# Sachin-A/TraceWeaver

Hardware: AMD Instinct MI355X
Metric: spans/sec reconstructed + assignment accuracy vs ground truth (higher is better)
Workload: dtype int64 timestamps, f64 scores; 1 GPU; media_microservices shape (6 services, E in {1,1,1,1,2,4}), 100000 requests/service x 16 replicas per GPU, concurrency 1.6, two-pass reconstruction, device mixture refit; spans_per_gpu=25600000, spans_total=25600000, parallelism=units sharded, 1 rank(s), backend none

## Files before the change

traceweaver_amd/csrc/tw_device.h:

```cpp
#pragma once
#include <hip/hip_runtime.h>
#include <stdint.h>

#include "traceweaver_amd.h"

namespace tw {

constexpr int kMaxEp = TW_MAX_EP;
constexpr int kTopK = TW_TOPK;
constexpr int kMaxComp = TW_MAX_COMP;
constexpr int kMaxWin = TW_MAX_WINDOW;
constexpr int kCandWords = TW_CAND_WORDS;
constexpr int kEnumStretches = 8;
constexpr int kTile = 128;
constexpr int kCoop = 256;
constexpr int32_t kNoOwner = 0x7f7f7f7f;

struct UnitDev {
    int64_t in_off;
    int64_t ie_off;
    int64_t ep_off[kMaxEp + 1];
    int32_t n_in;
    int32_t E;
    int32_t nblk;
// ... 91 lines not shown
    int32_t *heavy_in_unit, *heavy_in_idx;
    int32_t* heavy_big_count;
    int32_t *heavy_big_unit, *heavy_big_idx;
    int32_t heavy_big_off[kMaxEp + 2];
    int32_t* heavy_big_part;
    int32_t* heavy_big_slot;
    int32_t part_off[kMaxEp + 2];
    int32_t split_twins;
    int32_t* part_used;
    int32_t defer_min_e;
    int32_t defer_cap;
    unsigned long long* defer_list;
    int32_t* defer_used;
    int32_t* defer_count;
    int32_t *part_lo, *part_hi;
    int32_t* part_lvl;
    int32_t* any_wide;
    int32_t* redo_count;
    int32_t* defer_refused;
    int32_t lean_min_e;
    int32_t tile_max_deep;
    int32_t lean_grid;
    int32_t tile_rank;
    double* pair_pool;
    int32_t* pair_busy;
    int32_t* fb_count;
    int32_t* fb_total;
    int32_t *fb_unit, *fb_idx, *fb_part, *fb_slot;
    int32_t* split_count;
    int32_t *split_unit, *split_idx, *split_slot, *split_parts;
    int32_t* part_n;
    int64_t* part_leaves;
    double* part_score;
    int32_t* part_idx;
    unsigned long long* part_bits;
    int32_t* part_logn;
    double* part_log_sc;
    unsigned long long* part_log_ix;
    int32_t* err;
    unsigned long long* prof;
};

__device__ __forceinline__ int32_t hi_word(double x) { return (int32_t)(__double_as_longlong(x) >> 32); }
__device__ __forceinline__ uint32_t lo_word(double x) { return (uint32_t)__double_as_longlong(x); }
__device__ __forceinline__ double with_hi(double x, int32_t hi) {
    return __longlong_as_double((long long)(((uint64_t)(uint32_t)hi << 32) | (uint64_t)lo_word(x)));
// ... 199 lines not shown
```

traceweaver_amd/csrc/tw_engine.hip:

```cpp
#include <algorithm>
#include <chrono>
#include <cmath>
#include <cstdio>
#include <cstdlib>
#include <cstring>
#include <functional>
#include <string>
#include <type_traits>
#include <vector>

#include <hip/hip_runtime.h>
#include <rocprim/rocprim.hpp>

#include "traceweaver_amd.h"
#include "tw_kernels.h"
#include "tw_fit.h"
#include "tw_eval.h"
#include "tw_skip.h"
#include "tw_load.h"
#include "tw_baselines.h"
#include "tw_stitch.h"
#include "tw_attr.h"
#include "tw_conf.h"
#include "tw_dist.h"
// ... 60 lines not shown
    hipEvent_t stretch_ev[kMaxEp + 1][kEnumStretches] = {}, stretch_done[kMaxEp + 1] = {};
    int enum_stretches = 1, stretch_min_tiles = 2048;
    int heavy_grid = 4096, select_grid = 0;
    int debug_lists = 0;
    int32_t first_lists[3][kMaxEp + 1] = {};
    hipEvent_t gate_ev = nullptr;
    int tile_gate = 0;
    int stage_min_tiles = 1024;
    int32_t *rank_in = nullptr, *rank_out = nullptr;
    bool class_params = false;
    int prio_min_e = 0, prio_high = 0;
    bool prio_any = false;
    int pipeline = 1;
    std::string err;
    int state = ST_EMPTY;
    int tile = kTile;
    int tile_threads = 2;
    int tile_single = 1;
    int tile_rank = 1;
    int block_params = 1;
    int tile_single_threads = 1;
    int tile_pair = 1;
    int tile_pair_threads = 2;
    int coop = kCoop;
    std::vector<UnitDev> units;
    std::vector<TileDev> tiles;
    std::vector<int64_t> gs_off_h;
    std::vector<void*> allocs;
    void* arena = nullptr;
    size_t arena_cap = 0;
    bool arena_open = false;
    std::vector<std::pair<std::function<void(void*)>, size_t>> arena_req;
    Dev P{};
    int64_t n_ie = 0, n_gp = 0, n_slots = 0, n_gaps = 0;
    PairVI* agg_pair = nullptr;
    int32_t *agg_i32 = nullptr, *agg_i32b = nullptr;
    uint32_t *seg_in = nullptr, *seg_out = nullptr;
    int n_seg_out = 0;
    void* sort_tmp = nullptr;
    size_t sort_tmp_bytes = 0;
    double* mix_p_dev = nullptr;
    int32_t* mix_n_dev = nullptr;
    double* mix_c_dev = nullptr;
    double* gaps_sorted = nullptr;
    double* fit_models = nullptr;
    double* fit_uval = nullptr;
// ... 305 lines not shown
    const int pool = E > 4 ? 2048 : (E > 1 ? kPairPoolPerEp * E : 1);
    const size_t pool_bytes = sizeof(double) * (size_t)pool;
    const size_t lean_bytes = sizeof(double) * (size_t)(2 * kMaxEp * kNarrow + e->lean_pool), lean_bytes_w = sizeof(double) * (size_t)(2 * kMaxEp * 64 * kCandWords + e->lean_pool);
    const bool lean = E >= P.lean_min_e && !e->skip_mode;
    const int cap = P.heavy_in_off[E + 1] - P.heavy_in_off[E];
    auto grid_for = [&](int known, int most) { return std::max(std::min(((known >= 0 ? known : cap) + kWorkChunk - 1) / kWorkChunk, most), 1); };
    auto narrow = [&](int part, int g) {
        if (lean) hipLaunchKernelGGL((k_enumerate_lean<kNarrow>), dim3(g), hb, lean_bytes, st, P, pass, mode, part, e->lean_pool, E, E);
        else hipLaunchKernelGGL((k_enumerate_heavy<E, kNarrow>), dim3(g), hb, pool_bytes, st, P, pass, mode, part, pool);
    };
    auto wide = [&](int part, int g) {
        if (lean) hipLaunchKernelGGL((k_enumerate_lean<64 * kCandWords>), dim3(g), hb, lean_bytes_w, st, P, pass, mode, part, e->lean_pool, E, E);
        else hipLaunchKernelGGL((k_enumerate_heavy<E, 64 * kCandWords>), dim3(g), hb, pool_bytes, st, P, pass, mode, part, pool);
    };
    bool stretched = false;
    if (mode == 0 && pass == 1 && e->class_params) {
        const TileSet S = class_tiles(e, E);
        (void)sort_ends(e, S, st);
        launch_block_params(e, E, st);
    }
    if (mode == 0) {
        const bool single = E == 1 && e->tile_single != 0;
        const bool pair = E == 2 && e->tile_pair != 0;
        const dim3 tile_block(e->tile >= 64 ? e->tile * (single ? e->tile_single_threads : (pair ? e->tile_pair_threads : e->tile_threads)) : e->tile);
        int sub = 1;
        while (sub < e->tile_sub_max && nt * sub < 512 && (e->tile / (sub * 2)) * (sub * 2) == e->tile && e->tile / (sub * 2) >= 8) sub *= 2;
        const int ns = (!lean && !e->skip_mode && !(E >= 3 && E >= P.defer_min_e) && e->cls_stream2[E] != nullptr)
                           ? std::max(std::min(e->enum_stretches, nt / e->stretch_min_tiles), 1) : 1;
        stretched = ns > 1;
        for (int j = 0; j < ns; j++) {
            const int t0 = (int)((int64_t)nt * j / ns), t1 = (int)((int64_t)nt * (j + 1) / ns);
            const int32_t* ids = e->tile_ids + e->tile_cls_off[E] + t0;
            const bool sub_tile = e->tile == kTile && e->tile / sub == kSubTileSpans;
            if constexpr (E == 1) {
                if (single && sub_tile) hipLaunchKernelGGL((k_enumerate_tile<1, kSubTileSpans, true>), dim3((t1 - t0) * sub), tile_block, 0, st, P, pass, ids, t1 - t0, sub);
                else if (single) hipLaunchKernelGGL((k_enumerate_tile<1, kTile, true>), dim3((t1 - t0) * sub), tile_block, 0, st, P, pass, ids, t1 - t0, sub);
            }
            if constexpr (E == 2) {
                if (pair && sub_tile) hipLaunchKernelGGL((k_enumerate_tile<2, kSubTileSpans, false, true>), dim3((t1 - t0) * sub), tile_block, 0, st, P, pass, ids, t1 - t0, sub);
                else if (pair) hipLaunchKernelGGL((k_enumerate_tile<2, kTile, false, true>), dim3((t1 - t0) * sub), tile_block, 0, st, P, pass, ids, t1 - t0, sub);
            }
            if (single || pair) {}
            else if (sub_tile)
                hipLaunchKernelGGL((k_enumerate_tile<E, kSubTileSpans>), dim3((t1 - t0) * sub), tile_block, 0, st, P, pass, ids, t1 - t0, sub);
            else
                hipLaunchKernelGGL((k_enumerate_tile<E>), dim3((t1 - t0) * sub), tile_block, 0, st, P, pass, ids, t1 - t0, sub);
            if (ns > 1) {
                hipLaunchKernelGGL(k_enum_snapshot, dim3(1), dim3(1), 0, st, P, E, j + 1);
                if (j + 1 < ns) {
                    hipStream_t s2 = e->cls_stream2[E];
                    (void)hipEventRecord(e->stretch_ev[E][j], st);
                    (void)hipStreamWaitEvent(s2, e->stretch_ev[E][j], 0);
                    hipLaunchKernelGGL((k_enumerate_heavy<E, kNarrow>), dim3(grid_for(-1, e->heavy_grid)), hb, pool_bytes, s2, P, pass, mode, (j + 1) << 8, pool);
                } else {
                    hipLaunchKernelGGL((k_enumerate_heavy<E, kNarrow>), dim3(grid_for(-1, e->heavy_grid)), hb, pool_bytes, st, P, pass, mode, (j + 1) << 8, pool);
                    (void)hipEventRecord(e->stretch_done[E], e->cls_stream2[E]);
                    (void)hipStreamWaitEvent(st, e->stretch_done[E], 0);
                }
            }
        }
        if (e->tile_gate > 0 && nt >= e->tile_gate) { (void)hipEventRecord(e->tile_ev[E], st); e->gate_ev = e->tile_ev[E]; }
    }
    if (n_narrow != 0 && !stretched) narrow(0, grid_for(n_narrow, e->heavy_grid));
    if (n_wide != 0) wide(0, grid_for(n_wide, 1024));
    if (mode == 0 && E >= 3 && E >= P.defer_min_e) { narrow(3, grid_for(-1, 4096)); if (n_wide != 0) wide(3, grid_for(-1, 1024)); }
// ... 443 lines not shown
    HIPCHK(hipMemcpyAsync(const_cast<UnitDev*>(P.units), e->units.data(), sizeof(UnitDev) * e->units.size(), hipMemcpyHostToDevice, e->stream));
    HIPCHK(hipStreamSynchronize(e->stream));
    e->state = ST_LOADED; e->pass1_done = false;
    drop_batch_order(e);
    for (int E = 0; E <= kMaxEp; E++) { e->wide_pass1[E] = -1; e->hard_pass1[E] = -1; e->split_pass1[E] = -1; }
    return TW_OK;
}

extern "C" {

int tw_create(int device_id, tw_engine** out) {
    if (out == nullptr) return TW_ERR_ARG;
    *out = nullptr;
    tw_engine* e = new tw_engine();
    e->device = device_id;
    e->tile = std::min(std::max(env_int("TW_TILE", kTile), 1), kTile);
    e->tile_threads = std::min(std::max(env_int("TW_TILE_THREADS", 2), 1), 4);
    e->tile_single = env_int("TW_TILE_SINGLE", 1);
    e->block_params = env_int("TW_BLOCK_PARAMS", 1);
    e->tile_rank = env_int("TW_TILE_RANK", 1) != 0 ? 1 : 0;
    e->tile_single_threads = std::min(std::max(env_int("TW_TILE_SINGLE_THREADS", 1), 1), 4);
    e->tile_pair = env_int("TW_TILE_PAIR", 1);
    e->tile_pair_threads = std::min(std::max(env_int("TW_TILE_PAIR_THREADS", 2), 1), 2);
    e->coop = std::min(std::max(env_int("TW_COOP_THREADS", kCoop), 1), kCoop);
    if (env_int("TW_SET_HW_QUEUES", 0) != 0) setenv("GPU_MAX_HW_QUEUES", "12", 0);
    hipError_t s = hipSetDevice(device_id);
    if (s == hipSuccess) s = hipStreamCreate(&e->stream);
    for (int i = 0; i < EV_COUNT && s == hipSuccess; i++) s = hipEventCreate(&e->ev[i]);
    for (int i = 0; i < SE_COUNT && s == hipSuccess; i++) s = hipEventCreate(&e->stage_ev[i]);
    const int prio_min_e = env_int("TW_PRIO_MIN_E", 0);
    int prio_least = 0, prio_greatest = 0;
    if (s == hipSuccess) s = hipDeviceGetStreamPriorityRange(&prio_least, &prio_greatest);
    e->prio_min_e = prio_min_e; e->prio_high = prio_greatest; e->prio_any = prio_greatest != prio_least;
    for (int i = 0; i <= kMaxEp + 1 && s == hipSuccess; i++) s = hipEventCreateWithFlags(&e->cls_ev[i], hipEventDisableTiming);
    if (s == hipSuccess) s = hipEventCreateWithFlags(&e->prep_ev, hipEventDisableTiming);
    for (int i = 0; i <= kMaxEp && s == hipSuccess; i++) {
        s = hipEventCreateWithFlags(&e->post_fork[i], hipEventDisableTiming);
        if (s == hipSuccess) s = hipEventCreateWithFlags(&e->tile_ev[i], hipEventDisableTiming);
        if (s == hipSuccess) s = hipEventCreateWithFlags(&e->post_done[i], hipEventDisableTiming);
        if (s == hipSuccess) s = hipEventCreateWithFlags(&e->stretch_done[i], hipEventDisableTiming);
        for (int j = 0; j < kEnumStretches && s == hipSuccess; j++) s = hipEventCreateWithFlags(&e->stretch_ev[i][j], hipEventDisableTiming);
        for (int j = 0; j < 3 && s == hipSuccess; j++) s = hipEventCreateWithFlags(&e->post_join[i][j], hipEventDisableTiming);
    }
    e->pipeline = env_int("TW_CLASS_PIPELINE", 1);
    e->sig_hash_bits = std::min(std::max(env_int("TW_SIG_HASH_BITS", 64), 1), 64);
    e->tile_gate = env_int("TW_TILE_GATE", 0);
// ... 209 lines not shown
    std::vector<uint32_t> seg_gap_dst_h(seg_gap_h.size());
    e->n_gap_scored = 0;
    for (size_t r = 0; r < seg_gap_h.size(); r++) { seg_gap_dst_h[r] = (uint32_t)e->n_gap_scored; e->n_gap_scored += seg_gap_end_h[r] - seg_gap_h[r]; }
    seg_in[(size_t)b->n_units] = (uint32_t)n_in_total;
    seg_out.push_back((uint32_t)n_out_total);
    e->n_seg_out = (int)seg_out.size() - 1;
    e->n_ie = ie; e->n_gp = gp; e->n_slots = slots; e->n_gaps = gaps;

    Dev& P = e->P;
    P = Dev{};
    P.n_units = b->n_units;
    P.n_tiles = (int32_t)e->tiles.size();
    P.tile_spans = e->tile;
    P.n_in_total = n_in_total;
    P.n_out_total = n_out_total;
    P.batch_size = b->batch_size;
    P.batch_mis = b->batch_size_mis;
    P.split_twins = env_int("TW_SPLIT_TWINS", 2);
    P.defer_min_e = env_int("TW_DEFER_MIN_E", 5);
    P.lean_min_e = env_int("TW_LEAN_MIN_E", 5);
    P.lean_grid = std::max(env_int("TW_LEAN_GRID", TW_LEAN_GRID), 1);
    P.tile_max_deep = std::min(std::max(env_int("TW_TILE_MAX_DEEP", kTileMax), 0), kTileMax);
    P.tile_rank = e->tile_rank;
    int rc;
    e->arena_req.clear();
    e->arena_open = true;
    UnitDev* d_units; TileDev* d_tiles; int64_t *d_is, *d_ie, *d_os, *d_oe, *d_gs;
    DEV_ALLOC(d_units, P.n_units); DEV_ALLOC(d_tiles, P.n_tiles);
    DEV_ALLOC(d_is, n_in_total); DEV_ALLOC(d_ie, n_in_total); DEV_ALLOC(d_os, n_out_total); DEV_ALLOC(d_oe, n_out_total);
    DEV_ALLOC(d_gs, P.n_units);
    DEV_ALLOC(P.in_end_sorted, n_in_total); DEV_ALLOC(P.out_end_sorted, n_out_total);
    DEV_ALLOC(P.gparam, gp * 4);
    DEV_ALLOC(e->mix_n_dev, slots); DEV_ALLOC(e->mix_p_dev, slots * kMaxComp * 3); DEV_ALLOC(e->mix_c_dev, slots * kMaxComp * 4);
    DEV_ALLOC(P.pm_val, n_in_total); DEV_ALLOC(P.pm_idx, n_in_total); DEV_ALLOC(P.pc, n_in_total + 1); DEV_ALLOC(P.seg, n_in_total);
    DEV_ALLOC(P.win_end, n_in_total); DEV_ALLOC(P.wid, n_in_total); DEV_ALLOC(P.w_last, n_in_total);
    DEV_ALLOC(P.unit_nwin, P.n_units); DEV_ALLOC(P.w_dirty, n_in_total); DEV_ALLOC(P.w_conf, n_in_total);
    DEV_ALLOC(P.tk_n, n_in_total); DEV_ALLOC(P.leaves, n_in_total); DEV_ALLOC(P.leaves0, n_in_total); DEV_ALLOC(P.chosen, n_in_total); DEV_ALLOC(P.rep, n_in_total);
    DEV_ALLOC(P.tkr_n, n_in_total);
    DEV_ALLOC(P.tk_idx, ie * kTopK); DEV_ALLOC(P.tkr_idx, ie * kTopK);
    DEV_ALLOC(P.tk_score, n_in_total * kTopK); DEV_ALLOC(P.tkr_score, n_in_total * kTopK);
    DEV_ALLOC(P.c_lo, ie); DEV_ALLOC(P.c_hi, ie); DEV_ALLOC(P.c_bits, ie * kCandWords); DEV_ALLOC(P.parent, ie);
    DEV_ALLOC(P.gone, ie * kCandWords); DEV_ALLOC(P.gone_valid, n_in_total); DEV_ALLOC(P.leaves_r, n_in_total);
    DEV_ALLOC(P.frontier, (int64_t)kFrontierSlots * 2 * kFrontierCap); 
    P.frontier_big_slots = (int32_t)std::min<int64_t>(std::max<int64_t>(n_in_total / 16384, kFrontierBigSlots), std::max(kFrontierBigSlots, 512));
    DEV_ALLOC(P.frontier_big, (int64_t)P.frontier_big_slots * 2 * kFrontierBigCap);
    DEV_ALLOC(P.pair_pool, (int64_t)kPairSlots * kPairSpill);
// ... 1812 lines not shown
```

traceweaver_amd/csrc/tw_tile.h:

```cpp
#pragma once

namespace tw {

#ifndef TW_TILE_MAX
#define TW_TILE_MAX 256
#endif
constexpr int kTileMax = TW_TILE_MAX;
#ifndef TW_TILE_REPLAY_MAX
#define TW_TILE_REPLAY_MAX 256
#endif
constexpr int kTileReplayMax = TW_TILE_REPLAY_MAX;
#ifndef TW_TILE_RANK_DIRECT
#define TW_TILE_RANK_DIRECT 32
#endif
constexpr int kRankDirect = TW_TILE_RANK_DIRECT;
constexpr int kRankMinLong = (kRankDirect & ~3) + 4;
constexpr int kRankBuckets = 5;
static_assert(kRankDirect >= 24, "the maxima and counters of a segment's long spans lie in one byte per tuple slot");
__device__ __forceinline__ uint32_t score_key32(double v) {
    const unsigned long long u = (unsigned long long)__double_as_longlong(v + 0.0);
    return (uint32_t)(((u >> 63) ? ~u : (u | (1ull << 63))) >> 32);
}
__device__ __forceinline__ int pos_base(unsigned long long pk, int e) {
    int acc = 0;
    for (int f = 0; f < e; f++) acc += (int)((pk >> (8 * f)) & 255ull);
    return acc;
}
#ifndef TW_TILE_ITEMS
#define TW_TILE_ITEMS 768
#define TW_TILE_GRID 1024
#endif
constexpr int kSubTileSpans = kTile / 8;
#ifndef TW_TILE_PAIR_ITEMS
#define TW_TILE_PAIR_ITEMS 512
#define TW_TILE_PAIR_GRID 1024
#endif
template <int E, int SPANS = kTile, bool PAIR = false>
struct TileCfg {
#ifdef TW_TILE_SMALL
    static constexpr int kSlice = 24, kItems = PAIR ? 2 * 32 : kMaxEp * 32, kGrid = kTileMax > 64 ? kTileMax : 64;
#else
    static constexpr int kSlice = SPANS < kTile ? 64 : (E <= 4 ? 192 : 160);
    static constexpr int kItems = SPANS < kTile ? kMaxEp * 32 : (PAIR ? TW_TILE_PAIR_ITEMS : TW_TILE_ITEMS);
    static constexpr int kGrid = SPANS < kTile ? (kTileMax > 512 ? kTileMax : 512) : (PAIR ? TW_TILE_PAIR_GRID : TW_TILE_GRID);
#endif
    static_assert(kItems >= (PAIR ? 2 : kMaxEp) * 32 && kGrid >= ((kTileMax + 3) & ~3) && kGrid % 4 == 0, "a single span must fit a segment");
};

__device__ __forceinline__ uint32_t div_small(uint32_t rest, uint32_t c) {
#ifdef TW_HOST_EMULATION
    const float rc = 1.0f / (float)c;
#else
    const float rc = __builtin_amdgcn_rcpf((float)c);
#endif
    return (uint32_t)(((float)rest + 0.5f) * rc);
}

__device__ __forceinline__ int fresh(int v) {
#ifndef TW_HOST_EMULATION
    asm volatile("" : "+v"(v));
#endif
    return v;
}

template <int GRID, int MINLONG>
struct SurvivorRanks {
    static constexpr int kLong = (GRID - MINLONG) / MINLONG + 1;
// ... 94 lines not shown
#ifndef TW_PROFILE_TILE_E
#define TW_PROFILE_TILE_E 4
#endif
#define TW_TILE_T0() long long _tp = wall_clock64(); const long long _tb = _tp; long long _ta[7] = {0, 0, 0, 0, 0, 0, 0}
#define TW_TILE_TICK(k) do { const long long _n = wall_clock64(); _ta[k] += _n - _tp; _tp = _n; } while (0)
#define TW_TILE_COUNT(k, v) do { if (E == TW_PROFILE_TILE_E && threadIdx.x == 0) atomicAdd((unsigned long long*)&P.prof[k], (unsigned long long)(v)); } while (0)
#define TW_TILE_FLUSH() do { if (E == TW_PROFILE_TILE_E && threadIdx.x == 0) { for (int _k = 0; _k < 7; _k++) atomicAdd((unsigned long long*)&P.prof[_k], (unsigned long long)_ta[_k]); \
    atomicAdd((unsigned long long*)&P.prof[7], (unsigned long long)(wall_clock64() - _tb)); atomicAdd((unsigned long long*)&P.prof[8], 1ull); } } while (0)
#else
#define TW_TILE_T0() do {} while (0)
#define TW_TILE_TICK(k) do {} while (0)
#define TW_TILE_COUNT(k, v) do {} while (0)
#define TW_TILE_FLUSH() do {} while (0)
#endif

#ifdef TW_HOST_EMULATION
#define TW_TILE_ATTR
#else
#ifndef TW_TILE_PAIR_WAVES
#define TW_TILE_PAIR_WAVES 4
#endif
#define TW_TILE_ATTR __attribute__((amdgpu_waves_per_eu(SINGLE ? 8 : (PAIR ? TW_TILE_PAIR_WAVES : (E <= 4 ? 4 : 2)))))
#endif
template <int E, int SPANS = kTile, bool SINGLE = false, bool PAIR = false>
__global__ void __launch_bounds__(4 * kTile) TW_TILE_ATTR k_enumerate_tile(Dev P, int pass, const int32_t* tile_ids, int n_tiles_e, int sub_tiles) {
    static_assert(!SINGLE || E == 1, "the lean path is the one of a single endpoint");
    static_assert(!PAIR || (E == 2 && !SINGLE), "the pair path is the one of two endpoints");
    if (*P.err != 0) return;
    typedef TileCfg<E, SPANS, PAIR> C;
    constexpr int SL = C::kSlice;
    const int vb = xcd_tile(blockIdx.x, n_tiles_e * sub_tiles);
    const int tile = tile_ids[vb / sub_tiles];
    const TileDev T = P.tiles[tile];
    const UnitDev& U = P.units[T.unit];
    const int t = threadIdx.x, nt = blockDim.x;
    const int sub_spans = P.tile_spans / sub_tiles, first = T.first + (vb % sub_tiles) * sub_spans;
    const int ns = min(sub_spans, min(P.tile_spans, U.n_in - T.first) - (vb % sub_tiles) * sub_spans);
    if (ns <= 0) return;
    __shared__ int32_t s_is[SPANS], s_ie[SPANS];
    __shared__ int32_t sl_st[E][SL], sl_en[E][SL];
    __shared__ int32_t s_A[E], s_B[E];
    __shared__ uint16_t s_lo[E][SPANS];
    __shared__ uint32_t s_cm[E][SPANS];
    __shared__ uint32_t s_bits[E][SPANS];
    __shared__ int32_t s_item0[SPANS + 1], s_grid0[SPANS + 1], s_leaves[SPANS];
    __shared__ uint8_t s_amb[SPANS];
    __shared__ unsigned long long s_cn[SPANS];
    __shared__ int32_t s_wtot[4 * kTile / 64][2];
    __shared__ double t_root[C::kItems], t_close[C::kItems];
    __shared__ uint16_t it_idx[C::kItems];
    __shared__ double g_sc[C::kGrid + (PAIR ? 4 : 0)];
    __shared__ uint8_t g_span[C::kGrid];
    __shared__ uint32_t g_aux[C::kGrid / 4];
    __shared__ int32_t s_segend, s_anyamb;
    const bool live = t < ns;
    const int i = first + (live ? t : 0);
    const int64_t base = P.in_start[U.in_off + first];
    const int64_t in_start = P.in_start[U.in_off + i], in_end = P.in_end[U.in_off + i];
    const int64_t* os[E];
    const int64_t* oe[E];
#pragma unroll
    for (int e = 0; e < E; e++) { os[e] = P.out_start + U.ep_off[e]; oe[e] = P.out_end + U.ep_off[e]; }
    for (int x = t; x < E; x += nt) { s_A[x] = 0x7fffffff; s_B[x] = 0; }
    uint32_t dag_pm[E], dag_np[E], dag_pl[E];
    uint32_t ordered = 0;
#pragma unroll
    for (int e = 0; e < E; e++) {
        dag_pm[e] = U.pred_mask[e];
        dag_np[e] = U.npred[e];
        uint32_t pk = 0;
#pragma unroll
        for (int j = 0; j < E; j++) pk |= (j < (int)dag_np[e] ? ((uint32_t)U.pred_list[e][j] | ((uint32_t)U.pred_prim[e][j] << 3)) : 0u) << (4 * j);
        dag_pl[e] = pk;
        ordered |= dag_pm[e];
    }
// ... 108 lines not shown
                } else {
                    int64_t prev = INT64_MIN;
                    for (int cx = lo[e]; cx <= hi[e]; cx++) {
                        const int64_t st = os[e][cx];
                        if (st >= in_start && oe[e][cx] <= in_end) { v++; twins |= st == prev; prev = st; }
                    }
                }
                if (hprod <= (1ll << 40)) hprod *= v;
                if (e == 0) first_cands = v;
            }
            if (twins && P.split_twins == 0) first_cands = 0;
            twins_any = twins;
            if (E >= P.lean_min_e) first_cands = 0;
            if (E >= 3 && E >= P.defer_min_e) {
                uint32_t any_order = 0;
#pragma unroll
                for (int e = 0; e < E; e++) any_order |= U.pred_mask[e];
                if (any_order != 0) first_cands = 0;
            }
        }
        heavy_append<E>(P, live && !mine && !wide, narrow, hprod > kBigProduct, T.unit, i, hprod, U.skip ? 0 : first_cands, twins_any);
    }
    const bool some = mine && !empty && prod > 0;
    int nitem = 0;
    unsigned long long cnpack = 0;
    if (live) {
#pragma unroll
        for (int e = 0; e < E; e++) {
            const int rel = lo[e] - s_A[e], c = some ? __popcll((unsigned long long)cm[e]) : 0;
            s_lo[e][t] = (uint16_t)(some ? rel : 0);
            s_cm[e][t] = some ? cm[e] : 0u;
            if constexpr (!SINGLE) s_bits[e][t] = 0u;
            nitem += c;
            cnpack |= (unsigned long long)c << (8 * e);
        }
        s_is[t] = (int32_t)iso; s_ie[t] = (int32_t)ieo;
        s_amb[t] = 0;
        if constexpr (!SINGLE) { s_cn[t] = cnpack; s_leaves[t] = (some && !ordered) ? (int)prod : 0; }
    }
    {
        int a = live ? nitem : 0, b = (!SINGLE && live && some) ? (PAIR ? (int)prod : (((int)prod + 3) & ~3)) : 0;
        const int lane = t & 63, wv = t >> 6;
        for (int off = 1; off < 64; off <<= 1) {
            const int a2 = __shfl_up(a, off);
            if (lane >= off) a += a2;
            if constexpr (!SINGLE) { const int b2 = __shfl_up(b, off); if (lane >= off) b += b2; }
        }
        if (lane == 63 || t == nt - 1) { s_wtot[wv][0] = a; if constexpr (!SINGLE) s_wtot[wv][1] = b; }
        group_sync();
        for (int w = 0; w < wv; w++) { a += s_wtot[w][0]; if constexpr (!SINGLE) b += s_wtot[w][1]; }
        if (live) { s_item0[t + 1] = a; if constexpr (!SINGLE) s_grid0[t + 1] = b; }
        if (t == 0) { s_item0[0] = 0; if constexpr (!SINGLE) s_grid0[0] = 0; }
        group_sync();
    }
    TW_TILE_TICK(2);
    Scorer S;
    S.pass = pass;
    S.mix_n = P.mix_n + U.slot_off;
    S.mix_c = P.mix_c + (int64_t)U.slot_off * kMaxComp * 4;
    auto span_of = [&](const int32_t* pre, int first, int last, int x) -> int {
        int a = first, b = last - 1;
        while (a < b) { const int mid = (a + b + 1) >> 1; if (pre[mid] <= x) a = mid; else b = mid - 1; }
        return a;
    };
    auto decode = [&](int s, int gi, int it_first, int32_t (&kx)[E], int32_t (&ix)[E]) {
        uint32_t rest = (uint32_t)gi;
        const unsigned long long pk = s_cn[s];
        int below[E], acc = s_item0[s] - it_first;
#pragma unroll
        for (int e = 0; e < E; e++) { below[e] = acc; acc += (int)((pk >> (8 * e)) & 255ull); }
#pragma unroll
        for (int e = E - 1; e >= 0; e--) {
            const uint32_t c = (uint32_t)((pk >> (8 * e)) & 255ull);
            const uint32_t q = c == 1 ? rest : div_small(rest, c);
            kx[e] = below[e] + (int32_t)(rest - q * c);
// ... 283 lines not shown
                for (int k = 0; k < kTopK; k++) { hs[k] = RH.s[k]; hx[k] = (uint16_t)RH.x[k]; }
                py_sort_desc(hs, hx, RH.n, [&](double sa, unsigned long long xa, double sb, unsigned long long xb) { return RH.lt(sa, xa, sb, xb, start_of); });
                const int si = first + tl;
                for (int k = 0; k < RH.n; k++) {
                    P.tk_score[tks_index(U, k, si)] = hs[k];
                    P.tk_idx[tk_index(U, k, 0, si)] = s_A[0] + (int)it_idx[ks + (int)(hx[k] & 255u)];
                    P.tk_idx[tk_index(U, k, 1, si)] = s_A[1] + (int)(it_idx[ks + c0 + (int)(hx[k] >> 8)] & 0x7fff);
                }
                s_amb[tl] = 0;
            }
            if (mine_here && !s_amb[tl]) {
                const int i = first + tl;
                const int64_t g = U.in_off + i;
                const int leaves = s_leaves[tl];
                P.tk_n[g] = leaves < kTopK ? leaves : kTopK;
                P.leaves[g] = leaves;
                if (pass == 1) P.leaves0[g] = leaves;
                P.rep[g] = 0;
                if (pass == 1) {
#pragma unroll
                    for (int e = 0; e < 2; e++) {
                        P.c_bits[ie_index(U, e, i) * kCandWords] = (uint64_t)(ordered ? s_bits[e][tl] : s_cm[e][tl]);
                        for (int w = 1; w < kCandWords; w++) P.c_bits[ie_index(U, e, i) * kCandWords + w] = 0;
                    }
                }
            }
            group_sync();
            TW_TILE_TICK(6);
            seg = send;
        }
        TW_TILE_FLUSH();
        const int te = fresh(t);
        heavy_append<E>(P, te < ns && s_mine[te] != 0 && s_amb[te] != 0, true, false, T.unit, first + (te < ns ? te : 0), 0, 0, false, te & 63);
        return;
    } else
    for (int seg = 0; seg < ns;) {
        typedef SurvivorRanks<C::kGrid, kRankMinLong> SR;
        constexpr bool kRankFits = SR::kAuxWords <= C::kGrid / 4 && C::kGrid * 4 <= C::kItems * 8 && C::kGrid <= 65536;
        static_assert(kRankBuckets == kTopK && C::kGrid <= C::kItems * 8, "a subset of slots per entry of the list; a rank per slot in t_root");
        uint8_t* const g_rank = reinterpret_cast<uint8_t*>(t_root);
        const bool compact = kRankFits && P.tile_rank != 0;
        if (compact) SR{g_aux, g_rank, nullptr, nullptr, g_sc, g_span, s_grid0, 0}.clear(fresh(t), nt);
        if (t == 0) { s_segend = ns; s_anyamb = 0; }
        group_sync();
        if (live && t >= seg && (s_item0[t + 1] - s_item0[seg] > C::kItems || s_grid0[t + 1] - s_grid0[seg] > C::kGrid)) atomicMin(&s_segend, t);
        group_sync();
// ... 210 lines not shown
```

Measured before the change: 1.382 billion spans/s.

## Add specialized quad tile enumeration path for three- and four-endpoint spans

Adds a QUAD specialization of the tile enumeration kernel for units with three or four endpoints, enabled by default. It precomputes per-item root and closing gap scores as a compacted job list, and prunes closing candidates that cannot be the last-ending endpoint. Scores per tuple then reuse these precomputed terms. The kernel also gets its own item and grid sizes and unpadded grid counts. This removes redundant per-tuple scoring for the E=4 service, at the cost of more shared memory, an extra prefix scan, and a large new code path that could diverge from the generic one in results.

```diff
diff --git a/traceweaver_amd/csrc/tw_device.h b/traceweaver_amd/csrc/tw_device.h
--- a/traceweaver_amd/csrc/tw_device.h
+++ b/traceweaver_amd/csrc/tw_device.h
@@ -137,6 +137,7 @@
     int32_t tile_max_deep;
     int32_t lean_grid;
     int32_t tile_rank;
+    int32_t tile_quad_close;
     double* pair_pool;
     int32_t* pair_busy;
     int32_t* fb_count;
diff --git a/traceweaver_amd/csrc/tw_engine.hip b/traceweaver_amd/csrc/tw_engine.hip
--- a/traceweaver_amd/csrc/tw_engine.hip
+++ b/traceweaver_amd/csrc/tw_engine.hip
@@ -106,6 +106,8 @@
     int tile_single_threads = 1;
     int tile_pair = 1;
     int tile_pair_threads = 2;
+    int tile_quad = 1;
+    int tile_quad_close = 1;
     int coop = kCoop;
     std::vector<UnitDev> units;
     std::vector<TileDev> tiles;
@@ -457,6 +459,7 @@
     if (mode == 0) {
         const bool single = E == 1 && e->tile_single != 0;
         const bool pair = E == 2 && e->tile_pair != 0;
+        const bool quad = (E == 3 || E == 4) && e->tile_quad != 0;
         const dim3 tile_block(e->tile >= 64 ? e->tile * (single ? e->tile_single_threads : (pair ? e->tile_pair_threads : e->tile_threads)) : e->tile);
         int sub = 1;
         while (sub < e->tile_sub_max && nt * sub < 512 && (e->tile / (sub * 2)) * (sub * 2) == e->tile && e->tile / (sub * 2) >= 8) sub *= 2;
@@ -475,7 +478,11 @@
                 if (pair && sub_tile) hipLaunchKernelGGL((k_enumerate_tile<2, kSubTileSpans, false, true>), dim3((t1 - t0) * sub), tile_block, 0, st, P, pass, ids, t1 - t0, sub);
                 else if (pair) hipLaunchKernelGGL((k_enumerate_tile<2, kTile, false, true>), dim3((t1 - t0) * sub), tile_block, 0, st, P, pass, ids, t1 - t0, sub);
             }
-            if (single || pair) {}
+            if constexpr (E == 3 || E == 4) {
+                if (quad && sub_tile) hipLaunchKernelGGL((k_enumerate_tile<E, kSubTileSpans, false, false, true>), dim3((t1 - t0) * sub), tile_block, 0, st, P, pass, ids, t1 - t0, sub);
+                else if (quad) hipLaunchKernelGGL((k_enumerate_tile<E, kTile, false, false, true>), dim3((t1 - t0) * sub), tile_block, 0, st, P, pass, ids, t1 - t0, sub);
+            }
+            if (single || pair || quad) {}
             else if (sub_tile)
                 hipLaunchKernelGGL((k_enumerate_tile<E, kSubTileSpans>), dim3((t1 - t0) * sub), tile_block, 0, st, P, pass, ids, t1 - t0, sub);
             else
@@ -965,6 +972,8 @@
     e->tile_single_threads = std::min(std::max(env_int("TW_TILE_SINGLE_THREADS", 1), 1), 4);
     e->tile_pair = env_int("TW_TILE_PAIR", 1);
     e->tile_pair_threads = std::min(std::max(env_int("TW_TILE_PAIR_THREADS", 2), 1), 2);
+    e->tile_quad = env_int("TW_TILE_QUAD", 1);
+    e->tile_quad_close = env_int("TW_TILE_QUAD_CLOSE", 1) != 0 ? 1 : 0;
     e->coop = std::min(std::max(env_int("TW_COOP_THREADS", kCoop), 1), kCoop);
     if (env_int("TW_SET_HW_QUEUES", 0) != 0) setenv("GPU_MAX_HW_QUEUES", "12", 0);
     hipError_t s = hipSetDevice(device_id);
@@ -1220,6 +1229,7 @@
     P.lean_grid = std::max(env_int("TW_LEAN_GRID", TW_LEAN_GRID), 1);
     P.tile_max_deep = std::min(std::max(env_int("TW_TILE_MAX_DEEP", kTileMax), 0), kTileMax);
     P.tile_rank = e->tile_rank;
+    P.tile_quad_close = e->tile_quad_close;
     int rc;
     e->arena_req.clear();
     e->arena_open = true;
diff --git a/traceweaver_amd/csrc/tw_tile.h b/traceweaver_amd/csrc/tw_tile.h
--- a/traceweaver_amd/csrc/tw_tile.h
+++ b/traceweaver_amd/csrc/tw_tile.h
@@ -35,14 +35,18 @@
 #define TW_TILE_PAIR_ITEMS 512
 #define TW_TILE_PAIR_GRID 1024
 #endif
-template <int E, int SPANS = kTile, bool PAIR = false>
+#ifndef TW_TILE_QUAD_ITEMS
+#define TW_TILE_QUAD_ITEMS 512
+#define TW_TILE_QUAD_GRID 1024
+#endif
+template <int E, int SPANS = kTile, bool PAIR = false, bool QUAD = false>
 struct TileCfg {
 #ifdef TW_TILE_SMALL
     static constexpr int kSlice = 24, kItems = PAIR ? 2 * 32 : kMaxEp * 32, kGrid = kTileMax > 64 ? kTileMax : 64;
 #else
     static constexpr int kSlice = SPANS < kTile ? 64 : (E <= 4 ? 192 : 160);
-    static constexpr int kItems = SPANS < kTile ? kMaxEp * 32 : (PAIR ? TW_TILE_PAIR_ITEMS : TW_TILE_ITEMS);
-    static constexpr int kGrid = SPANS < kTile ? (kTileMax > 512 ? kTileMax : 512) : (PAIR ? TW_TILE_PAIR_GRID : TW_TILE_GRID);
+    static constexpr int kItems = SPANS < kTile ? kMaxEp * 32 : (PAIR ? TW_TILE_PAIR_ITEMS : (QUAD ? TW_TILE_QUAD_ITEMS : TW_TILE_ITEMS));
+    static constexpr int kGrid = SPANS < kTile ? (kTileMax > 512 ? kTileMax : 512) : (PAIR ? TW_TILE_PAIR_GRID : (QUAD ? TW_TILE_QUAD_GRID : TW_TILE_GRID));
 #endif
     static_assert(kItems >= (PAIR ? 2 : kMaxEp) * 32 && kGrid >= ((kTileMax + 3) & ~3) && kGrid % 4 == 0, "a single span must fit a segment");
 };
@@ -183,12 +187,13 @@
 #endif
 #define TW_TILE_ATTR __attribute__((amdgpu_waves_per_eu(SINGLE ? 8 : (PAIR ? TW_TILE_PAIR_WAVES : (E <= 4 ? 4 : 2)))))
 #endif
-template <int E, int SPANS = kTile, bool SINGLE = false, bool PAIR = false>
+template <int E, int SPANS = kTile, bool SINGLE = false, bool PAIR = false, bool QUAD = false>
 __global__ void __launch_bounds__(4 * kTile) TW_TILE_ATTR k_enumerate_tile(Dev P, int pass, const int32_t* tile_ids, int n_tiles_e, int sub_tiles) {
     static_assert(!SINGLE || E == 1, "the lean path is the one of a single endpoint");
     static_assert(!PAIR || (E == 2 && !SINGLE), "the pair path is the one of two endpoints");
     if (*P.err != 0) return;
-    typedef TileCfg<E, SPANS, PAIR> C;
+    static_assert(!QUAD || ((E == 3 || E == 4) && !SINGLE && !PAIR), "the quad path is the one of three and four endpoints");
+    typedef TileCfg<E, SPANS, PAIR, QUAD> C;
     constexpr int SL = C::kSlice;
     const int vb = xcd_tile(blockIdx.x, n_tiles_e * sub_tiles);
     const int tile = tile_ids[vb / sub_tiles];
@@ -205,13 +210,14 @@
     __shared__ uint32_t s_cm[E][SPANS];
     __shared__ uint32_t s_bits[E][SPANS];
     __shared__ int32_t s_item0[SPANS + 1], s_grid0[SPANS + 1], s_leaves[SPANS];
+    __shared__ int32_t s_job0[QUAD ? SPANS + 1 : 1];
     __shared__ uint8_t s_amb[SPANS];
     __shared__ unsigned long long s_cn[SPANS];
-    __shared__ int32_t s_wtot[4 * kTile / 64][2];
+    __shared__ int32_t s_wtot[4 * kTile / 64][QUAD ? 3 : 2];
     __shared__ double t_root[C::kItems], t_close[C::kItems];
     __shared__ uint16_t it_idx[C::kItems];
-    __shared__ double g_sc[C::kGrid + (PAIR ? 4 : 0)];
-    __shared__ uint8_t g_span[C::kGrid];
+    __shared__ double g_sc[C::kGrid + (PAIR || QUAD ? 4 : 0)];
+    __shared__ uint8_t g_span[C::kGrid] __attribute__((aligned(4)));
     __shared__ uint32_t g_aux[C::kGrid / 4];
     __shared__ int32_t s_segend, s_anyamb;
     const bool live = t < ns;
@@ -366,8 +372,36 @@
         heavy_append<E>(P, live && !mine && !wide, narrow, hprod > kBigProduct, T.unit, i, hprod, U.skip ? 0 : first_cands, twins_any);
     }
     const bool some = mine && !empty && prod > 0;
-    int nitem = 0;
+    int nitem = 0, njob = 0;
     unsigned long long cnpack = 0;
+    uint32_t clm[QUAD ? E : 1];
+    if constexpr (QUAD) {
+#pragma unroll
+        for (int e = 0; e < E; e++) clm[e] = some ? cm[e] : 0u;
+        if (some && !ordered && P.tile_quad_close != 0) {
+            int32_t mn[E];
+#pragma unroll
+            for (int e = 0; e < E; e++) {
+                const int rel = lo[e] - s_A[e];
+                mn[e] = 0x7fffffff;
+                for (uint32_t m = cm[e]; m != 0; m &= m - 1) { const int32_t en = sl_en[e][rel + __ffs((int)m) - 1]; mn[e] = en < mn[e] ? en : mn[e]; }
+            }
+#pragma unroll
+            for (int e = 0; e < E; e++) {
+                const int rel = lo[e] - s_A[e];
+                int32_t above = -0x7fffffff - 1, reach = -0x7fffffff - 1;
+#pragma unroll
+                for (int f = 0; f < E; f++) { if (f < e && mn[f] > above) above = mn[f]; if (f > e && mn[f] > reach) reach = mn[f]; }
+                uint32_t keep = 0;
+                for (uint32_t m = cm[e]; m != 0; m &= m - 1) {
+                    const int r = __ffs((int)m) - 1;
+                    const int32_t en = sl_en[e][rel + r];
+                    if (en > above && en >= reach) keep |= 1u << r;
+                }
+                clm[e] = keep;
+            }
+        }
+    }
     if (live) {
 #pragma unroll
         for (int e = 0; e < E; e++) {
@@ -375,6 +409,10 @@
             s_lo[e][t] = (uint16_t)(some ? rel : 0);
             s_cm[e][t] = some ? cm[e] : 0u;
             if constexpr (!SINGLE) s_bits[e][t] = 0u;
+            if constexpr (QUAD) {
+                if (!ordered) s_bits[e][t] = clm[e];
+                njob += (dag_np[e] == 0 ? c : 0) + __popcll((unsigned long long)clm[e]);
+            }
             nitem += c;
             cnpack |= (unsigned long long)c << (8 * e);
         }
@@ -383,18 +421,21 @@
         if constexpr (!SINGLE) { s_cn[t] = cnpack; s_leaves[t] = (some && !ordered) ? (int)prod : 0; }
     }
     {
-        int a = live ? nitem : 0, b = (!SINGLE && live && some) ? (PAIR ? (int)prod : (((int)prod + 3) & ~3)) : 0;
+        int a = live ? nitem : 0, b = (!SINGLE && live && some) ? (PAIR || QUAD ? (int)prod : (((int)prod + 3) & ~3)) : 0;
+        int c = live ? njob : 0;
         const int lane = t & 63, wv = t >> 6;
         for (int off = 1; off < 64; off <<= 1) {
             const int a2 = __shfl_up(a, off);
             if (lane >= off) a += a2;
             if constexpr (!SINGLE) { const int b2 = __shfl_up(b, off); if (lane >= off) b += b2; }
-        }
-        if (lane == 63 || t == nt - 1) { s_wtot[wv][0] = a; if constexpr (!SINGLE) s_wtot[wv][1] = b; }
+            if constexpr (QUAD) { const int c2 = __shfl_up(c, off); if (lane >= off) c += c2; }
+        }
+        if (lane == 63 || t == nt - 1) { s_wtot[wv][0] = a; if constexpr (!SINGLE) s_wtot[wv][1] = b; if constexpr (QUAD) s_wtot[wv][2] = c; }
         group_sync();
-        for (int w = 0; w < wv; w++) { a += s_wtot[w][0]; if constexpr (!SINGLE) b += s_wtot[w][1]; }
-        if (live) { s_item0[t + 1] = a; if constexpr (!SINGLE) s_grid0[t + 1] = b; }
-        if (t == 0) { s_item0[0] = 0; if constexpr (!SINGLE) s_grid0[0] = 0; }
+        for (int w = 0; w < wv; w++) { a += s_wtot[w][0]; if constexpr (!SINGLE) b += s_wtot[w][1]; if constexpr (QUAD) c += s_wtot[w][2]; }
+        if (live) { s_item0[t + 1] = a; if constexpr (!SINGLE) s_grid0[t + 1] = b; if constexpr (QUAD) s_job0[t + 1] = c; }
+        if (t == 0) { s_item0[0] = 0; if constexpr (!SINGLE) s_grid0[0] = 0; if constexpr (QUAD) s_job0[0] = 0; }
+        (void)c;
         group_sync();
     }
     TW_TILE_TICK(2);
@@ -724,6 +765,268 @@
                     for (int e = 0; e < 2; e++) {
                         P.c_bits[ie_index(U, e, i) * kCandWords] = (uint64_t)(ordered ? s_bits[e][tl] : s_cm[e][tl]);
                         for (int w = 1; w < kCandWords; w++) P.c_bits[ie_index(U, e, i) * kCandWords + w] = 0;
+                    }
+                }
+            }
+            group_sync();
+            TW_TILE_TICK(6);
+            seg = send;
+        }
+        TW_TILE_FLUSH();
+        const int te = fresh(t);
+        heavy_append<E>(P, te < ns && s_mine[te] != 0 && s_amb[te] != 0, true, false, T.unit, first + (te < ns ? te : 0), 0, 0, false, te & 63);
+        return;
+    } else if constexpr (QUAD) {
+        static_assert(SL <= 256 && E <= 4, "the slice positions of a tuple's candidates lie in a byte each of 32 bits");
+        static_assert(C::kItems <= (1 << 14), "an item's number in 15 bits of a job, its endpoint above 14 bits of it_idx");
+        __shared__ uint8_t it_span[C::kItems];
+        __shared__ uint32_t g_ix[C::kGrid];
+        __shared__ uint8_t s_row[C::kGrid / 64 + 1];
+        __shared__ uint8_t s_mine[SPANS];
+        if (live) s_mine[t] = mine ? 1 : 0;
+        uint16_t* const jobs = reinterpret_cast<uint16_t*>(g_sc);
+        constexpr int kJobs = 2 * C::kItems < 4 * C::kGrid ? 2 * C::kItems : 4 * C::kGrid;
+        static_assert(kJobs >= 2 * E * 32, "the jobs of a single span must fit a segment");
+        typedef SurvivorRanks<C::kGrid, kRankDirect + 1> SR;
+        constexpr bool kRankFits = SR::kAuxWords <= C::kGrid / 4 && C::kGrid * 4 <= C::kItems * 8 && C::kGrid <= 65536;
+        static_assert(C::kGrid <= C::kItems * 8, "a rank per slot in t_root");
+        uint8_t* const g_rank = reinterpret_cast<uint8_t*>(t_root);
+        const bool compact = kRankFits && P.tile_rank != 0;
+        const bool scan = (nt & 63) == 0;
+        for (int seg = 0; seg < ns;) {
+            if (compact) SR{g_aux, g_rank, nullptr, nullptr, g_sc, g_span, s_grid0, 0}.clear(fresh(t), nt);
+            for (int x = fresh(t); x < C::kGrid / 4; x += nt) reinterpret_cast<uint32_t*>(g_span)[x] = 0u;
+            if (t == 0) { s_segend = ns; s_anyamb = 0; }
+            group_sync();
+            if (live && t >= seg && (s_item0[t + 1] - s_item0[seg] > C::kItems || s_grid0[t + 1] - s_grid0[seg] > C::kGrid || (kJobs < 2 * C::kItems && s_job0[t + 1] - s_job0[seg] > kJobs))) atomicMin(&s_segend, t);
+            group_sync();
+            const int send = s_segend;
+            const int it0 = s_item0[seg], nIt = s_item0[send] - it0, g0 = s_grid0[seg], nG = s_grid0[send] - g0, j0 = s_job0[seg], nJ = s_job0[send] - j0;
+            const SR sr{g_aux, g_rank, reinterpret_cast<uint16_t*>(t_close), reinterpret_cast<uint16_t*>(t_close) + C::kGrid, g_sc, g_span, s_grid0, g0};
+            const int tq = fresh(t);
+            const bool here = tq < ns && tq >= seg && tq < send;
+            TW_TILE_TICK(2);
+            TW_TILE_COUNT(9, 1); TW_TILE_COUNT(10, nIt); TW_TILE_COUNT(11, nG); TW_TILE_COUNT(12, nJ);
+            if (here) {
+                int k = s_item0[tq] - it0, j = s_job0[tq] - j0;
+#pragma unroll
+                for (int e = 0; e < E; e++) {
+                    const int rel = s_lo[e][tq];
+                    const bool is_root = dag_np[e] == 0;
+                    const uint32_t cl = ordered ? s_cm[e][tq] : s_bits[e][tq];
+                    for (uint32_t m = s_cm[e][tq]; m != 0; m &= m - 1, k++) {
+                        const int r = __ffs((int)m) - 1;
+                        it_span[k] = (uint8_t)tq;
+                        it_idx[k] = (uint16_t)((rel + r) | (e << 14));
+                        if (is_root) jobs[j++] = (uint16_t)k;
+                        if ((cl >> r) & 1u) jobs[j++] = (uint16_t)(k | 0x8000);
+                        else t_close[k] = dnan();
+                    }
+                }
+                const int gs = s_grid0[tq] - g0, ge = s_grid0[tq + 1] - g0;
+                if (ge > gs) {
+                    g_span[gs] = (uint8_t)tq;
+                    for (int r = (gs + 63) >> 6; (r << 6) < ge; r++) s_row[r] = (uint8_t)tq;
+                }
+            }
+            group_sync();
+            for (int j = t; j < nJ; j += nt) {
+                const int jb = jobs[j], k = jb & 0x7fff;
+                const bool closing = (jb >> 15) != 0;
+                const int s = it_span[k], e = it_idx[k] >> 14, idx = it_idx[k] & 255;
+                const long long gap = closing ? (long long)s_ie[s] - sl_en[e][idx] : (long long)sl_st[e][idx] - s_is[s];
+                S.gp = P.gparam + (U.gp_off + (int64_t)((first + s) / P.batch_size) * U.nslot) * 4;
+                const double v = score_term_gap(S, closing ? slot_close(E, e) : slot_root(E, e), gap);
+                (closing ? t_close : t_root)[k] = v;
+            }
+            group_sync();
+            TW_TILE_TICK(3);
+            for (int gb = 0; gb < nG; gb += nt) {
+                const int g = gb + t;
+                int s = 0;
+                if (scan) {
+                    const int lane = t & 63;
+                    if (g < nG) { s = g_span[g]; if (lane == 0) { const int c = s_row[g >> 6]; s = c > s ? c : s; } }
+                    for (int off = 1; off < 64; off <<= 1) { const int s2 = __shfl_up(s, off); if (lane >= off && s2 > s) s = s2; }
+                } else if (g < nG) s = span_of(s_grid0, seg, send, g0 + g);
+                if (g >= nG) continue;
+                const int gi = g - (s_grid0[s] - g0);
+                const uint32_t pk = (uint32_t)s_cn[s];
+                int32_t kx[E], ix[E], st[E], en[E];
+                {
+                    uint32_t rest = (uint32_t)gi;
+                    int below[E], acc = s_item0[s] - it0;
+#pragma unroll
+                    for (int e = 0; e < E; e++) { below[e] = acc; acc += (int)((pk >> (8 * e)) & 255u); }
+#pragma unroll
+                    for (int e = E - 1; e >= 0; e--) {
+                        const uint32_t c = (pk >> (8 * e)) & 255u;
+                        const uint32_t q = e == 0 ? 0u : (c == 1 ? rest : div_small(rest, c));
+                        kx[e] = below[e] + (int32_t)(rest - q * c);
+                        rest = q;
+                        ix[e] = it_idx[kx[e]] & 255;
+                    }
+                }
+                bool ok = true;
+#pragma unroll
+                for (int e = 0; e < E; e++) {
+                    st[e] = sl_st[e][ix[e]]; en[e] = sl_en[e][ix[e]];
+#pragma unroll
+                    for (int p = 0; p < e; p++)
+                        if (((dag_pm[e] >> p) & 1) && en[p] > st[e]) ok = false;
+                }
+                double sj = 0.0;
+                if (ok) {
+                    int last = 0;
+                    int32_t last_end = en[0];
+#pragma unroll
+                    for (int e = 1; e < E; e++) if (en[e] > last_end) { last_end = en[e]; last = e; }
+                    if (ordered) S.gp = P.gparam + (U.gp_off + (int64_t)((first + s) / P.batch_size) * U.nslot) * 4;
+#pragma unroll
+                    for (int e = 0; e < E; e++) {
+                        const int np = (int)dag_np[e];
+#pragma unroll
+                        for (int j = 0; j < E; j++) {
+                            if (j >= np) continue;
+                            const uint32_t pj = (dag_pl[e] >> (4 * j)) & 15u;
+                            if (!(pj & 8u)) continue;
+                            const int p = (int)(pj & 7u);
+                            int32_t pend = 0;
+#pragma unroll
+                            for (int q = 0; q < E; q++) if (q == p) pend = en[q];
+                            sj += score_term_gap(S, fresh(slot_prim(E, p, e)), (long long)st[e] - pend);
+                        }
+                        if (np == 0) sj += t_root[kx[e]];
+                        if (e == last) sj += t_close[kx[e]];
+                    }
+                    if (ordered) {
+                        atomicAdd(&s_leaves[s], 1);
+                        if (pass == 1) {
+#pragma unroll
+                            for (int e = 0; e < E; e++) atomicOr(&s_bits[e][s], 1u << (ix[e] - (int)s_lo[e][s]));
+                        }
+                    }
+                }
+                uint32_t ixp = 0;
+#pragma unroll
+                for (int e = 0; e < E; e++) ixp |= (uint32_t)ix[e] << (8 * e);
+                g_sc[g] = ok ? sj : dnan();
+                g_ix[g] = ixp;
+                g_span[g] = (uint8_t)s;
+                if (compact && ok && s_grid0[s + 1] - s_grid0[s] > kRankDirect) sr.note(g, gi, sj);
+            }
+            group_sync();
+            TW_TILE_TICK(4);
+            auto order_equal = [&](uint32_t a, uint32_t b) -> int {
+                const uint32_t d = a ^ b;
+                const int e = d == 0u ? 0 : (__ffs((int)d) - 1) >> 3;
+                const int32_t sa = sl_st[e][(a >> (8 * e)) & 255u], sb = sl_st[e][(b >> (8 * e)) & 255u];
+                return sb > sa ? 1 : (sb < sa ? -1 : 0);
+            };
+            if (compact) sr.collect(nG, fresh(t), nt);
+            for (int g = t; g < nG; g += nt) {
+                const double my = g_sc[g];
+                int rank = kTopK;
+                const int s = g_span[g];
+                const int gs = s_grid0[s] - g0, ge = s_grid0[s + 1] - g0;
+                if (compact && ge - gs > kRankDirect) { g_rank[g] = (uint8_t)kTopK; continue; }
+                if (my == my) {
+                    rank = 0;
+                    bool partner = false;
+                    int eq = 0;
+                    for (int h0 = gs; h0 < ge && rank < kTopK; h0 += 4) {
+                        const double o0 = g_sc[h0], o1 = g_sc[h0 + 1], o2 = g_sc[h0 + 2], o3 = g_sc[h0 + 3];
+                        const bool in1 = h0 + 1 < ge, in2 = h0 + 2 < ge, in3 = h0 + 3 < ge;
+                        rank += (o0 > my) + (in1 && o1 > my) + (in2 && o2 > my) + (in3 && o3 > my);
+                        eq += (o0 == my) + (in1 && o1 == my) + (in2 && o2 == my) + (in3 && o3 == my);
+                    }
+                    if (eq > 1 && rank < kTopK) {
+                        const uint32_t mine_ix = g_ix[g];
+                        for (int h = gs; h < ge; h++) {
+                            if (h == g || !(g_sc[h] == my)) continue;
+                            const int ord = order_equal(mine_ix, g_ix[h]);
+                            if (ord > 0) rank++;
+                            else if (ord == 0) partner = true;
+                        }
+                    }
+                    if (partner && rank < kTopK) { s_amb[s] = 1; s_anyamb = 1; }
+                }
+                g_rank[g] = (uint8_t)(rank < kTopK ? rank : kTopK);
+            }
+            if (compact) {
+                group_sync();
+                sr.rank(fresh(t), nt,
+                        [&](int s, int gi) -> uint32_t { return g_ix[s_grid0[s] - g0 + gi]; },
+                        [&](int s, uint32_t mine_ix, int hrel) { return order_equal(mine_ix, g_ix[s_grid0[s] - g0 + hrel]); },
+                        [&](int s) { s_amb[s] = 1; s_anyamb = 1; });
+            }
+            group_sync();
+            TW_TILE_TICK(5);
+            for (int g = t; g < nG; g += nt) {
+                if (g_rank[g] >= kTopK) continue;
+                const int s = g_span[g];
+                if (s_amb[s]) continue;
+                const int k = g_rank[g], si = first + s;
+                const uint32_t ixp = g_ix[g];
+                P.tk_score[tks_index(U, k, si)] = g_sc[g];
+#pragma unroll
+                for (int e = 0; e < E; e++) P.tk_idx[tk_index(U, k, e, si)] = s_A[e] + (int)((ixp >> (8 * e)) & 255u);
+            }
+            if (s_anyamb != 0) group_sync();
+            const int tl = fresh(t);
+            const bool mine_here = tl < ns && tl >= seg && tl < send && s_mine[tl] != 0;
+            const int th = tl < SPANS / 2 ? tl : tl - SPANS / 2;
+            const bool replay = s_anyamb != 0 && mine_here && s_amb[tl] && (th + 1) * (kTopK + 1) <= C::kItems && (tl + 1) * (kTopK + 1) <= C::kGrid && s_leaves[tl] <= kTileReplayMax;
+            if (replay) {
+                const int ks = s_item0[tl] - it0;
+                const uint32_t pk = (uint32_t)s_cn[tl];
+                auto start_of = [&](int e, int pos) -> int32_t { return sl_st[e][it_idx[ks + pos_base((unsigned long long)pk, e) + pos] & 255]; };
+                RegHeap RH;
+                RH.clear(E);
+                const int gs = s_grid0[tl] - g0, nT = s_grid0[tl + 1] - s_grid0[tl];
+                uint32_t x = 0;
+                for (int gi = 0; gi < nT; gi++) {
+                    const double sc = g_sc[gs + gi];
+                    const uint32_t xc = x;
+                    {
+                        bool carry = true;
+#pragma unroll
+                        for (int e = E - 1; e >= 0; e--) {
+                            if (!carry) continue;
+                            const uint32_t c = (pk >> (8 * e)) & 255u, d = (x >> (8 * e)) & 255u;
+                            if (d + 1 < c) { x += 1u << (8 * e); carry = false; } else x &= ~(255u << (8 * e));
+                        }
+                    }
+                    if (!(sc == sc) || RH.below_root(sc)) continue;
+                    RH.push(sc, (unsigned long long)xc, start_of);
+                }
+                double* hs = (tl < SPANS / 2 ? t_root : t_close) + th * (kTopK + 1);
+                uint32_t* hx = g_ix + tl * (kTopK + 1);
+#pragma unroll
+                for (int k = 0; k < kTopK; k++) { hs[k] = RH.s[k]; hx[k] = (uint32_t)RH.x[k]; }
+                py_sort_desc(hs, hx, RH.n, [&](double sa, unsigned long long xa, double sb, unsigned long long xb) { return RH.lt(sa, xa, sb, xb, start_of); });
+                const int si = first + tl;
+                for (int k = 0; k < RH.n; k++) {
+                    P.tk_score[tks_index(U, k, si)] = hs[k];
+#pragma unroll
+                    for (int e = 0; e < E; e++)
+                        P.tk_idx[tk_index(U, k, e, si)] = s_A[e] + (int)(it_idx[ks + pos_base((unsigned long long)pk, e) + (int)((hx[k] >> (8 * e)) & 255u)] & 255);
+                }
+                s_amb[tl] = 0;
+            }
+            if (mine_here && !s_amb[tl]) {
+                const int i1 = first + tl;
+                const int64_t g = U.in_off + i1;
+                const int leaves = s_leaves[tl];
+                P.tk_n[g] = leaves < kTopK ? leaves : kTopK;
+                P.leaves[g] = leaves;
+                if (pass == 1) P.leaves0[g] = leaves;
+                P.rep[g] = 0;
+                if (pass == 1) {
+#pragma unroll
+                    for (int e = 0; e < E; e++) {
+                        P.c_bits[ie_index(U, e, i1) * kCandWords] = (uint64_t)(ordered ? s_bits[e][tl] : s_cm[e][tl]);
+                        for (int w = 1; w < kCandWords; w++) P.c_bits[ie_index(U, e, i1) * kCandWords + w] = 0;
                     }
                 }
             }
```

Measured after the change: 1.378 billion spans/s. Within noise of the previous version (-0.3%).
